# cmower/optas

Measured on AMD Instinct MI355X. Metric: MPC solves/sec (KUKA 7-DoF, T=50), higher is better.
Workload: dtype f64; 1 GPU; figure_eight_plan T=50 KUKA LWR end_effector_ball (BASELINE configs[1]) x 262144 perturbed instances per GPU (qc0 + U(-0.1,0.1)^7, seed=qc), solved to reduced-gradient tol 1e-08, max_iter 300; batch_per_gpu=262144, global_batch=262144, T=50, parallelism=dp1 (instances sharded, one RCCL broadcast of constants), rccl_world=1, hessian=hybrid, streams_per_gpu=2

## Files before the change

optas_amd/csrc/oh_api.hip:

```cpp
#include <algorithm>
#include <chrono>
#include <cmath>
#include <cstdlib>
#include <cstring>
#include <string>
#include <thread>
#include <utility>
#include <vector>

#include "oh_handle.h"

static thread_local std::string g_err;

int fail(int code, const std::string& msg) {
  g_err = msg;
  return code;
}

extern "C" int oh_specialize(oh_handle* h);
static bool spec_applies(const oh_handle* h);
static bool spec_tail_vel_applies(const oh_handle* h);
extern "C" const char* oh_last_error(void) { return g_err.c_str(); }
extern "C" const char* oh_version(void) { return "optas_hip 0.2 (gfx950)"; }
extern "C" int oh_abi_version(void) { return OH_ABI_VERSION; }

struct FieldOpt {
  const char* name;
  int Sched::*i;
  double Sched::*d = nullptr;
  bool flag = false;
  double get(const Sched& s) const { return d ? s.*d : s.*i; }
  void set(Sched& s, const double v) const { if (d) s.*d = v; else s.*i = flag ? v != 0.0 : (int)v; }
};
static const FieldOpt FIELD_OPTS[] = {
    {"tail_threshold", &Sched::tail_threshold}, {"free_pcr_max", &Sched::free_pcr_max}, {"compaction", &Sched::compaction, nullptr, true},
    {"compact_frac", nullptr, &Sched::compact_frac}, {"compact_sort", &Sched::compact_sort}, {"compact_carry", &Sched::compact_carry},
    {"compact_fused", &Sched::compact_fused, nullptr, true},
    {"tail_vel", &Sched::tail_vel}, {"lg_split", &Sched::lg_split}, {"tail_vel_threshold", &Sched::tail_vel_threshold},
    {"fuse_couple", &Sched::fuse_couple, nullptr, true}, {"sparse_check_below", &Sched::sparse_check_below}, {"specialize", &Sched::specialize},
    {"tq_check", &Sched::tq_check},
};
static const FieldOpt* field_opt(const std::string& name) {
  for (const FieldOpt& f : FIELD_OPTS)
    if (name == f.name) return &f;
  return nullptr;
}
static int set_option_impl(oh_handle* h, const std::string& name, double v) {
  Sched& sc = h->sch;
  if (name == "compact_frac") sc.compact_frac = sc.compact_frac_restart = v;
  else if (name == "specialize") sc.specialize = v == 0.0 ? OH_SPECIALIZE_NEVER : (v == 1.0 ? OH_SPECIALIZE_ALWAYS : OH_SPECIALIZE_AUTO);
  else if (name == "tq_check") sc.tq_check = v >= 1.0 ? (int)v : 1;
  else if (name == "batch_invariant") {
// ... 551 lines not shown
  for (int i = 1; i <= S; ++i) lo[i] = (int)((long long)a.B * i / S / 64 * 64);
  lo[S] = a.B;
  std::vector<LastSolve::Part> parts(S);
  const int rc = fan_out(h, S, [&](const int i, oh_handle* q, Tally& t) {
    parts[i] = {q, lo[i + 1] - lo[i]};
    return lane_solve(q, t, a.part((size_t)lo[i], parts[i].n, sh));
  });
  if (rc) return rc;
  rec->parts = parts;
  return OH_OK;
}

struct Traj {
  int B, N, NV, check_every, hard_cap;
  bool guarded, lead, prof, invariant;
  const FigSpec* spec;
  FreeSweep sweep;
  const double* p;
  double *x, *f, *kkt;
  int *iters, *status;
  int launched, compactions;
  size_t ne;
};
static FreeSweep free_sweep(oh_handle* h, const int nb, const bool start = false) {
  const int N = h->desc.ndof, nK = h->desc.T - h->P.t0;
  FreeSweep sw = FREE_SERIAL;
  if (!h->P.lock && batch_invariant(h) == 0.0 && nb <= h->sch.free_pcr_max && nK <= 128 && (N == 6 || N == 7)) {
    if (N == 7 && (int)optv(h, "free_bb") != 0) sw = FREE_BB;
    else sw = (nb <= (int)optv(h, "free_cp_max") && nK <= 64) ? FREE_CP : FREE_PCR;
  }
// ... 13 lines not shown
}
static bool check_after(const oh_handle* h, const Traj& r, const int it, const bool tail_ok) {
  return (it + 1) % ((!tail_ok && r.check_every == 1 && h->D.B <= h->sch.sparse_check_below) ? 8 : r.check_every) == 0;
}
static int look(oh_handle* h, const bool check, int* nrun) {
  *nrun = -1;
  if (!check) return OH_OK;
  hipStream_t s = h->stream;
  HIPCHK(hipMemcpyAsync(h->h_flag, h->D.n_running, sizeof(int), hipMemcpyDeviceToHost, s));
  HIPCHK(hipStreamSynchronize(s));
  *nrun = *h->h_flag;
  return OH_OK;
}
static void finalize(oh_handle* h, const Traj& r, const int only_done) {
  hipStream_t s = h->stream;
  if (r.spec && r.spec->finalize) {
    oh_launch_finalize(s, r.N, h->P, h->D, only_done, r.x, r.f, r.kkt, r.iters, r.status, 1);
    if (oh_spec_launch_finalize(*r.spec, s, h->P, h->D, only_done, r.f, r.kkt, r.iters, r.status) == hipSuccess) return;
    (void)hipGetLastError();
    oh_launch_finalize(s, r.N, h->P, h->D, only_done, r.x, r.f, r.kkt, r.iters, r.status, 2);
    return;
  }
  oh_launch_finalize(s, r.N, h->P, h->D, only_done, r.x, r.f, r.kkt, r.iters, r.status);
}
static int compact_batch(oh_handle* h, Traj& r, const int nrun, const int slot, const bool move) {
  hipStream_t s = h->stream;
  finalize(h, r, 1);
  if (r.guarded) oh_launch_guard_emit(s, h->P, h->D, h->GP, h->GB, r.NV, 1);
  oh_launch_scan_running(s, h->D, h->sch.compact_sort);
  if (move) {
// ... 15 lines not shown
    bool want = h->sch.specialize == OH_SPECIALIZE_ALWAYS || (h->sch.specialize == OH_SPECIALIZE_AUTO && r.B >= h->specialize_min_B);
    if (!want && h->sch.specialize == OH_SPECIALIZE_AUTO && !h->spec_cache_checked) {
      h->spec_cache_checked = true;
      want = oh_jit_figure8_cached(h->chain_host, h->desc.ndof);
    }
    if (want && oh_specialize(h) != OH_OK) h->spec_failed = true;
  }
  if (r.lead && (r.guarded || !h->desc.lock_orientation || h->desc.ndof != 6))
    return fail(OH_ERR_INVALID, "oh_solve_device: a parameterised lead joint is lowered for the orientation-locked family with 6 optimised joints, "
                                "without inequality rows");
  if (!r.guarded) h->D.fpsi = nullptr;
  else if (const int rc = ensure_guards(h)) return rc;
  r.sweep = free_sweep(h, r.B, true);
  r.NV = (r.guarded && h->GP.vel) ? 2 * r.N : 0;
  r.spec = spec_applies(h) ? h->spec : nullptr;
  r.check_every = optv(h, "check_every") >= 1.0 ? (int)optv(h, "check_every") : 1;
  r.hard_cap = 2 * h->desc.max_iter + 2 + 40 + 64;
  hipStream_t s = h->stream;
  if (r.prof) {
    const size_t need = 4 * (size_t)(2 * h->desc.max_iter + 44) + 64;
    while (h->prof_events.size() < need) {
      hipEvent_t e;
      HIPCHK(hipEventCreate(&e));
      h->prof_events.push_back(e);
    }
  }
  HIPCHK(hipEventRecord(h->ev0, s));
  HIPCHK(hipMemsetAsync(h->D.work, 0, 4 * sizeof(unsigned long long), s));
  if (!oh_launch_setup(s, r.N, h->P, h->D, x0, r.p)) return fail(OH_ERR_INVALID, "oh_solve_device: unsupported ndof");
  if (r.guarded) oh_launch_setup_guards(s, r.N, h->P, h->D, h->GP, h->GB, r.p);
  h->prof_tags.clear();
  return mark(h, r, 0);
}
static bool launch_tail(oh_handle* h, const Traj& r, const bool tail_vel, const int slot) {
  hipStream_t s = h->stream;
  if (tail_vel && h->spec && spec_tail_vel_applies(h)) return oh_spec_launch_tail_vel(*h->spec, s, h->P, h->D, h->GP, h->GB, slot) == hipSuccess;
  if (tail_vel) return oh_launch_tail_vel(s, r.N, h->P, h->D, h->GP, h->GB, slot);
  if (r.spec) return oh_spec_launch_tail(*r.spec, s, h->P, h->D, slot) == hipSuccess;
  return oh_launch_tail(s, r.N, h->P, h->D, slot);
}
static void launch_eval(oh_handle* h, const Traj& r, const int slot, const int part) {
  if (!r.spec) oh_launch_eval(h->stream, r.N, h->P, h->D, slot, part);
  else oh_spec_launch_eval(*r.spec, h->stream, h->P, h->D, slot, part);
}
// ... 122 lines not shown
    if (nrun == 0) break;
    if (nrun > 0 && h->sch.compaction && D.B >= 512 && (double)nrun <= h->sch.compact_frac_restart * (double)D.B) {
      if (const int rc = compact_batch(h, r, nrun, (it + 1) & 1, false)) return rc;
      sweep = free_sweep(h, D.B);
      h->free_sweeps_used |= 1 << (int)sweep;
      if (const int rc = mark(h, r, 0)) return rc;
    }
  }
  return OH_OK;
}
static int traj_epilogue(oh_handle* h, Traj& r) {
  hipStream_t s = h->stream;
  finalize(h, r, 0);
  if (r.guarded) oh_launch_guard_emit(s, h->P, h->D, h->GP, h->GB, r.NV, 0);
  h->D.B = r.B;
  if (r.guarded) oh_launch_guard_infeasible(s, r.N, h->P, h->D, h->GP, r.p, r.B, r.kkt, r.status);
  if (const int frc = finish_solve(h, r.launched)) return frc;
  unsigned long long work[3] = {0, 0, 0};
  HIPCHK(hipMemcpyAsync(work, h->D.work, sizeof(work), hipMemcpyDeviceToHost, s));
  HIPCHK(hipStreamSynchronize(s));
  h->timing[6] = (double)work[0];
  h->rejects = (double)work[1];
  h->tail_iters = (double)work[2];
  if (r.prof) {
    double ms[4] = {0, 0, 0, 0};
    int n[5] = {0, 0, 0, 0, 0};
    for (size_t i = 1; i < r.ne; ++i) {
      const int tag = h->prof_tags[i];
      float m = 0.f;
      if (tag) hipEventElapsedTime(&m, h->prof_events[i - 1], h->prof_events[i]);
// ... 345 lines not shown
```

optas_amd/csrc/oh_figure8_kernels.h:

```cpp
#pragma once
#include "oh_figure8_units.h"

template <int N, bool MOVE = false>
__device__ void retract_block(const FigParams& P, const FigBuffers& D, const int slot) {
  eval_unit<N, false, false, EVAL_RETRACT_ONLY, false, true, MOVE>(P, D, slot, blockIdx.x * blockDim.x + threadIdx.x, blockIdx.y + P.t0);
}
template <int N>
__device__ void finalize_block(const FigParams& P, const FigBuffers& D, const int only_done, double* __restrict__ f, double* __restrict__ kkt, int* __restrict__ iters,
                               int* __restrict__ status) {
  finalize_unit<N>(P, D, only_done, nullptr, f, kkt, iters, status, blockIdx.x * blockDim.x + threadIdx.x, blockIdx.y);
}
template <int N, bool ZC = false>
__device__ void evalb_block(const FigParams& P, const FigBuffers& D, const int slot) {
  if constexpr (ZC) {
    if (blockIdx.x == 0 && threadIdx.x == 0) *D.n_running = 0;
    const int Tn = P.T - P.t0;
    const int w = blockIdx.x;
    const int chunk = w / (8 * Tn), r = w - chunk * 8 * Tn;
    eval_unit<N, false, false, EVAL_ONLY, true>(P, D, slot, (chunk * 8 + (r & 7)) * blockDim.x + threadIdx.x, (r >> 3) + P.t0);
  } else {
    eval_unit<N, false, false, EVAL_ONLY, false>(P, D, slot, blockIdx.x * blockDim.x + threadIdx.x, blockIdx.y + P.t0);
  }
}

OH_DEV double bcast(const double v, const int lane) {
// ... 526 lines not shown
```

optas_amd/csrc/oh_figure8_units.h:

```cpp
#pragma once
#include "oh_figure8.h"

#define IDX(t, K, k) (((size_t)(t) * (K) + (k)) * Bp + b)
#define KNOT(arr, t, K) rowbuf((arr) + (size_t)(t) * (K) * (size_t)Bp)
#define RB(k) ((unsigned)(k) * rowB)
#define SPARE(k) (((size_t)t * N + (k)) * Bp + nb)



template <int N>
OH_DEV void setup_unit(const FigParams& P, const FigBuffers& D, const double* __restrict__ x0, const double* __restrict__ pin, const int b, const int tt) {
  const int Bp = D.Bp;
  if (b >= D.B) {
    if (b < Bp && tt == 0) D.status[b] = OH_STATUS_CONVERGED;
    return;
  }
  const oh_chain* ch = D.chain;
  double qc[N];
#pragma unroll
  for (int j = 0; j < N; ++j) qc[j] = pin[(size_t)b * P.np + j];
#pragma unroll
  for (int j = 0; j < N; ++j) {
    const double v = (tt < P.t0) ? qc[j] : x0[(size_t)b * P.nx + (size_t)tt * N + j];
    D.q[0][IDX(tt, N, j)] = v;
    D.q[1][IDX(tt, N, j)] = (tt < P.t0) ? qc[j] : 0.0;
  }
  if (ch->has_lead) D.lead[(size_t)tt * Bp + b] = pin[(size_t)b * P.np + N + 1 + tt];
  if (tt != 0) return;
  double R[9], p[3], z[N][3], pj[N][3];
  if (ch->has_lead) {
    double Rb[9], pb[3];
    lead_base(ch, pin[(size_t)b * P.np + N], Rb, pb);
    fk_chain<N, true>(ch, qc, R, p, z, pj, Rb, pb);
  } else {
    fk_chain<N>(ch, qc, R, p, z, pj);
  }
  double e[3], t[3], Re[9];
  mv3(R, ch->p_tool, t);
  e[0] = p[0] + t[0]; e[1] = p[1] + t[1]; e[2] = p[2] + t[2];
  mm3(R, ch->R_tool, Re);
#pragma unroll
  for (int i = 0; i < 3; ++i) D.ref[(size_t)i * Bp + b] = e[i];
#pragma unroll
// ... 1039 lines not shown
#pragma unroll
      for (int a = 0; a < NZ; ++a) {
        rb_st(KNOT(D.zstep, t, NZ), RB(a), lb, alpha * zz[a]);
        z2 += zz[a] * zz[a];
      }
    }
    D.pred[b] = -alpha * gd + 0.5 * alpha * alpha * (gd + mu * z2);
  }
  D.mu[b] = mu;
  D.iters[b] = iters + 1;
  return true;
}


template <int N>
OH_DEV void knot_multipliers(const FigParams& P, const FigBuffers& D, const int b, const int t, const int cur, double* out) {
  const int Bp = D.Bp;
  if (t < P.t0) {
    out[0] = out[1] = out[2] = out[3] = 0.0;
    return;
  }
  const oh_chain* ch = OH_CHAIN(D);
  const double* __restrict__ qs = D.q[cur];
  const double kap2 = 2.0 * P.kappa;
  double q[N], G[N];
  const bool last = (t == P.T - 1);
#pragma unroll
  for (int k = 0; k < N; ++k) {
    q[k] = qs[IDX(t, N, k)];
    if (P.zc) {
      G[k] = D.Gfull[cur][IDX(t, N, k)];
    } else {
      G[k] = D.g[cur][IDX(t, N, k)] + kap2 * (q[k] - qs[IDX(t - 1, N, k)]);
      if (!last) G[k] -= kap2 * (qs[IDX(t + 1, N, k)] - q[k]);
    }
  }
  double R[9], p[3], z[N][3], pj[N][3];
  if (ch->has_lead) {
    double Rb[9], pb[3];
    lead_base(ch, D.lead[(size_t)t * Bp + b], Rb, pb);
    fk_chain<N, true>(ch, q, R, p, z, pj, Rb, pb);
  } else {
    fk_chain<N>(ch, q, R, p, z, pj);
  }
  double S[6] = {1e-14, 0, 1e-14, 0, 0, 1e-14};
  double rhs[3] = {0, 0, 0};
#pragma unroll
  for (int k = 0; k < N; ++k) {
    if (ch->jtype[k] == 0) {
      S[0] += z[k][0] * z[k][0];
      S[1] += z[k][1] * z[k][0];
      S[2] += z[k][1] * z[k][1];
      S[3] += z[k][2] * z[k][0];
      S[4] += z[k][2] * z[k][1];
      S[5] += z[k][2] * z[k][2];
      rhs[0] -= z[k][0] * G[k]; rhs[1] -= z[k][1] * G[k]; rhs[2] -= z[k][2] * G[k];
    }
  }
  chol_packed<3>(S, 0.0);
  fsub<3>(S, rhs);
  bsub<3>(S, rhs);
  double quat[4] = {0, 0, 0, 1};
#pragma unroll
  for (int k = 0; k < N; ++k) {
    double qn[4];
    qmul(quat, ch->quat0[k], qn);
    if (ch->jtype[k] == 0) {
      double sh, chh;
      sincos_joint(0.5 * qs[IDX(0, N, k)], &sh, &chh);
      const double qa[4] = {sh * ch->axis[k][0], sh * ch->axis[k][1], sh * ch->axis[k][2], chh};
      qmul(qn, qa, quat);
    } else {
      quat[0] = qn[0]; quat[1] = qn[1]; quat[2] = qn[2]; quat[3] = qn[3];
    }
  }
  double qcq[4];
  qmul(quat, ch->quat_tool, qcq);
  const double o[4] = {rhs[0], rhs[1], rhs[2], 0.0};
  double nu[4];
  qmul(o, qcq, nu);
  out[0] = -2.0 * nu[0]; out[1] = -2.0 * nu[1]; out[2] = -2.0 * nu[2]; out[3] = -2.0 * nu[3];
}

template <int N>
OH_DEV void finalize_unit(const FigParams& P, const FigBuffers& D, int only_done, double* __restrict__ x, double* __restrict__ f,
                          double* __restrict__ kkt, int* __restrict__ iters, int* __restrict__ status, const int b, const int t) {
  const int Bp = D.Bp;
  if (b >= D.B) return;
  const int st = D.status[b];
  if (only_done && st < 0) return;
  const size_t ob = (size_t)D.orig[b];
  const int cur = D.cur[b];
  const double* __restrict__ qs = D.q[cur];
  if (x) {
    double* xb = x + ob * P.nx;
    double q0[N];
// ... 28 lines not shown
```

optas_amd/csrc/oh_handle.h:

```cpp
#pragma once
#include <hip/hip_runtime.h>

#include <array>
#include <map>
#include <string>
#include <vector>

#include "oh_kernels.h"
#include "oh_carve.h"
#include "oh_jit.h"

int fail(int code, const std::string& msg);

#define HIPCHK(expr)                                                                                   \
  do {                                                                                                 \
    hipError_t _e = (expr);                                                                            \
    if (_e != hipSuccess) {                                                                            \
      return fail(OH_ERR_HIP, std::string(#expr) + ": " + hipGetErrorString(_e));                     \
    }                                                                                                  \
  } while (0)

#define OH_PINNED_STAGE_BYTES (256 * 1024)

template <class T, bool PINNED = false>
// ... 28 lines not shown
struct Solve {
  int B;
  const double *x0, *p;
  double *x, *f, *kkt;
  int *iters, *status;
  Solve part(const size_t lo, const int n, const Shape& sh) const {
    const auto at = [lo](auto* q, const size_t per) -> decltype(q) { return q ? q + lo * per : nullptr; };
    return {n, at(x0, sh.nx), at(p, sh.npar), at(x, sh.nx), at(f, 1), at(kkt, 3), at(iters, 1), at(status, 1)};
  }
};

struct Sched {
  int compaction = 1;
  int compact_carry = 1;
  int compact_fused = 1;
  int tail_vel_threshold = 1 << 30;
  int lg_split = 1;
  int tail_vel = 1;
  int compact_sort = 1;
  double compact_frac = 0.97;
  double compact_frac_restart = 0.9;
  int tail_threshold = 16384;
  int sparse_check_below = 2048;
  int fuse_couple = 1;
  int free_pcr_max = 1536;
  int specialize = OH_SPECIALIZE_AUTO;
  int tq_check = 4;
  std::array<double, 4> inv_saved{1.0, 16384.0, 1.0, -2.0};
};

// ... 193 lines not shown
```

optas_amd/csrc/oh_jit.h:

```cpp
#pragma once
#include <string>
#include <vector>

#include "oh_kernels.h"

struct FigSpec {
  hipModule_t mod = nullptr;
  hipFunction_t retract = nullptr, retract_move = nullptr, evalb = nullptr, evalb_zc = nullptr, tail = nullptr, tail_vel = nullptr, finalize = nullptr;
  int n = 0;
  bool from_disk = false;
  double seconds = 0.0;
};
std::string oh_jit_figure8_source(const oh_chain& chain, int N);
int oh_jit_compile_cached(const std::string& src, std::vector<char>* code, bool* from_disk, std::string* err, bool ignore_disk = false);
int oh_jit_figure8(const oh_chain& chain, int N, const FigSpec** out, std::string* err);
bool oh_jit_figure8_cached(const oh_chain& chain, int N);
hipError_t oh_spec_launch_eval(const FigSpec& sp, hipStream_t s, const FigParams& P, const FigBuffers& D, int slot, int part);
hipError_t oh_spec_launch_tail(const FigSpec& sp, hipStream_t s, const FigParams& P, const FigBuffers& D, int slot);
hipError_t oh_spec_launch_finalize(const FigSpec& sp, hipStream_t s, FigParams P, FigBuffers D, int only_done, double* f, double* kkt, int* iters, int* status);
hipError_t oh_spec_launch_tail_vel(const FigSpec& sp, hipStream_t s, FigParams P, FigBuffers D, GuardParams GP, GuardBuffers GB, int slot);
bool oh_spec_kernel_info(const FigSpec& sp, const char* name, OhKernelInfo* out);

bool oh_jit_disk_lookup(const std::string& key_text, const char* prefix, std::vector<char>* code);
void oh_jit_disk_store(const std::string& key_text, const char* prefix, const std::vector<char>& code);
void oh_jit_disk_drop(const std::string& key_text, const char* prefix);

struct FkSpec {
  hipModule_t mod = nullptr;
  hipFunction_t soa = nullptr, aos = nullptr;
  int ndof = 0;
  bool from_disk = false;
  double seconds = 0.0;
};
std::string oh_jit_fkjac_source(const oh_chain& chain);
// ... 4 lines not shown
```

optas_amd/csrc/oh_jit.hip:

```cpp
#include <hip/hip_runtime.h>
#include <hip/hiprtc.h>
#include <sys/stat.h>
#include <unistd.h>

#include <chrono>
#include <cstdio>
#include <cstdlib>
#include <cstring>
#include <map>
#include <mutex>
#include <string>
#include <vector>

#include "oh_jit.h"
#include "oh_fkjac_unit.h"
#include "oh_jit_headers.h"

namespace {
std::mutex g_mutex;
std::map<unsigned long long, FigSpec*> g_specs;
std::map<unsigned long long, FkSpec*> g_fk_specs;

unsigned long long fnv1a(const std::string& s, unsigned long long h = 1469598103934665603ull) {
  for (unsigned char c : s) {
// ... 165 lines not shown
  s += "#define OH_RETRACT_PREFETCH " + std::to_string(OH_JIT_RETRACT_PREFETCH) + "\n";
#ifndef OH_JIT_ZC_EARLY
#define OH_JIT_ZC_EARLY 1
#endif
  s += "#define OH_ZC_EARLY " + std::to_string(OH_JIT_ZC_EARLY) + "\n";
  s += "#include \"oh_platform_gfx950.h\"\n";
  s += "#include \"oh_figure8_kernels.h\"\n";
  const std::string n = std::to_string(N);
  s += "extern \"C\" __global__ __launch_bounds__(256, 2) void oh_spec_retract(FigParams P, FigBuffers D, const int slot) { retract_block<" + n + ">(P, D, slot); }\n";
  s += "extern \"C\" __global__ __launch_bounds__(256, 2) void oh_spec_retract_move(FigParams P, FigBuffers D, const int slot) { retract_block<" + n + ", true>(P, D, slot); }\n";
  s += "extern \"C\" __global__ __launch_bounds__(256, 2) void oh_spec_evalb(FigParams P, FigBuffers D, const int slot) { evalb_block<" + n + ">(P, D, slot); }\n";
  s += "extern \"C\" __global__ __launch_bounds__(256, 2) void oh_spec_evalb_zc(FigParams P, FigBuffers D, const int slot) { evalb_block<" + n + ", true>(P, D, slot); }\n";
  s += "extern \"C\" __global__ __launch_bounds__(64) void oh_spec_tail(FigParams P, FigBuffers D, const int slot) { tail_block<" + n + ">(P, D, slot); }\n";
  s += "extern \"C\" __global__ __launch_bounds__(256) void oh_spec_finalize(FigParams P, FigBuffers D, const int only_done, double* f, double* kkt, int* iters, int* status) { finalize_block<" + n +
       ">(P, D, only_done, f, kkt, iters, status); }\n";
  s += "extern \"C\" __global__ __launch_bounds__(64) void oh_spec_tail_vel(FigParams P, FigBuffers D, GuardParams GP, GuardBuffers GB, const int slot) { tail_block<" + n +
       ", true>(P, D, slot, &GP, &GB); }\n";
  return s;
}

int oh_jit_compile_cached(const std::string& src, std::vector<char>* code, bool* from_disk, std::string* err, bool ignore_disk) {
  const std::string name = cache_name(src);
  const std::string dir = cache_dir();
  *from_disk = false;
  if (ignore_disk && !dir.empty()) remove((dir + "/" + name).c_str());
  if (!ignore_disk && !dir.empty() && read_file(dir + "/" + name, code)) {
    *from_disk = true;
    return 0;
  }
  if (compile(src, code, err)) return 1;
// ... 34 lines not shown
    return 0;
  }
  std::vector<char> code;
  bool from_disk = false;
  FigSpec* sp = new FigSpec();
  for (int attempt = 0;; ++attempt) {
    if (oh_jit_compile_cached(src, &code, &from_disk, err, attempt > 0)) {
      delete sp;
      return 1;
    }
    const char* what = nullptr;
    if (hipModuleLoadData(&sp->mod, code.data()) != hipSuccess) what = "hipModuleLoadData";
    else if (hipModuleGetFunction(&sp->retract, sp->mod, "oh_spec_retract") != hipSuccess || hipModuleGetFunction(&sp->evalb, sp->mod, "oh_spec_evalb") != hipSuccess ||
             hipModuleGetFunction(&sp->tail, sp->mod, "oh_spec_tail") != hipSuccess || hipModuleGetFunction(&sp->evalb_zc, sp->mod, "oh_spec_evalb_zc") != hipSuccess ||
             hipModuleGetFunction(&sp->tail_vel, sp->mod, "oh_spec_tail_vel") != hipSuccess || hipModuleGetFunction(&sp->finalize, sp->mod, "oh_spec_finalize") != hipSuccess ||
             hipModuleGetFunction(&sp->retract_move, sp->mod, "oh_spec_retract_move") != hipSuccess) {
      what = "hipModuleGetFunction";
      hipModuleUnload(sp->mod);
    }
    if (!what) break;
    (void)hipGetLastError();
    if (from_disk && attempt == 0) continue;
    *err = std::string(what) + " failed for the specialised figure-eight kernels";
    delete sp;
    return 1;
  }
  sp->n = N;
  sp->from_disk = from_disk;
  sp->seconds = std::chrono::duration<double>(std::chrono::steady_clock::now() - t0).count();
  g_specs.emplace(key, sp);
  *out = sp;
// ... 9 lines not shown
  hipError_t e = hipSuccess;
  if (part == 3) return launch3(sp.retract_move, ge, dim3(256), s, P, D, slot);
  if (part != 2) e = launch3(sp.retract, ge, dim3(256), s, P, D, slot);
  if (e == hipSuccess && part != 1) {
    if (P.zc) e = launch3(sp.evalb_zc, dim3((((D.B + 255) / 256) + 7) / 8 * 8 * (P.T - P.t0)), dim3(256), s, P, D, slot);
    else e = launch3(sp.evalb, ge, dim3(256), s, P, D, slot);
  }
  return e;
}
hipError_t oh_spec_launch_tail(const FigSpec& sp, hipStream_t s, const FigParams& P, const FigBuffers& D, int slot) {
  return launch3(sp.tail, dim3(D.B), dim3(64), s, P, D, slot);
}
hipError_t oh_spec_launch_finalize(const FigSpec& sp, hipStream_t s, FigParams P, FigBuffers D, int only_done, double* f, double* kkt, int* iters, int* status) {
  void* args[] = {&P, &D, &only_done, &f, &kkt, &iters, &status};
  return hipModuleLaunchKernel(sp.finalize, (D.B + 255) / 256, D.lam_h ? P.T : 1, 1, 256, 1, 1, 0, s, args, nullptr);
}
hipError_t oh_spec_launch_tail_vel(const FigSpec& sp, hipStream_t s, FigParams P, FigBuffers D, GuardParams GP, GuardBuffers GB, int slot) {
  void* args[] = {&P, &D, &GP, &GB, &slot};
  return hipModuleLaunchKernel(sp.tail_vel, D.B, 1, 1, 64, 1, 1, 0, s, args, nullptr);
}
bool oh_spec_kernel_info(const FigSpec& sp, const char* name, OhKernelInfo* out) {
  const std::string n(name);
  hipFunction_t f = n == "k_retract" ? sp.retract : n == "k_retract_move" ? sp.retract_move : n == "k_evalb" ? sp.evalb : n == "k_evalb_zc" ? sp.evalb_zc : n == "k_tail" ? sp.tail : n == "k_tail_vel" ? sp.tail_vel : nullptr;
  if (!f) return false;
  int v = 0, sc = 0, lds = 0;
  if (hipFuncGetAttribute(&v, HIP_FUNC_ATTRIBUTE_NUM_REGS, f) != hipSuccess) return false;
  hipFuncGetAttribute(&sc, HIP_FUNC_ATTRIBUTE_LOCAL_SIZE_BYTES, f);
  hipFuncGetAttribute(&lds, HIP_FUNC_ATTRIBUTE_SHARED_SIZE_BYTES, f);
  out->vgprs = v;
  out->scratch_bytes = sc;
// ... 77 lines not shown
```

optas_amd/csrc/oh_kernels.h:

```cpp
#pragma once
#include <hip/hip_runtime.h>

#include <string>
#include <vector>

#include "optas_hip.h"
#include "oh_types.h"

struct OhKernelInfo {
  int vgprs, scratch_bytes, lds_bytes, block, blocks_per_cu;
};
bool oh_kernel_info_figure8(const char* name, OhKernelInfo* out);
bool oh_kernel_info_fkjac(const char* name, OhKernelInfo* out);
bool oh_kernel_info_torque(const char* name, OhKernelInfo* out);
bool oh_kernel_info_linkkin(const char* name, OhKernelInfo* out);
bool oh_kernel_info_qp_block(const char* name, OhKernelInfo* out);

void oh_launch_fk_jac(hipStream_t s, bool soa, const oh_chain* d_chain, int n_chain, int ndof, int n, const double* q, double* pose, double* J);
struct OhLinkFrames {
  oh_chain link, base;
  int n_shared;
};
void oh_launch_link_kin(hipStream_t s, bool soa, const OhLinkFrames* d_frames, int n_link, int n, const double* q, const double* a3, const oh_link_out& out);
bool oh_launch_setup(hipStream_t s, int n, const FigParams& P, const FigBuffers& D, const double* x0, const double* p);
bool oh_launch_eval(hipStream_t s, int n, const FigParams& P, const FigBuffers& D, int slot, int part = 0);
bool oh_launch_carry(hipStream_t s, int n, const FigParams& P, const FigBuffers& D, int phase, int Bnew, int slot);
bool oh_launch_eval_lead(hipStream_t s, int n, const FigParams& P, const FigBuffers& D, int slot);
bool oh_launch_couple(hipStream_t s, int n, const FigParams& P, const FigBuffers& D, int slot);
bool oh_launch_couple_vel(hipStream_t s, int n, const FigParams& P, const FigBuffers& D, const GuardParams& GP, const GuardBuffers& GB, int slot);
bool oh_launch_step(hipStream_t s, int n, const FigParams& P, const FigBuffers& D, int slot);
bool oh_launch_eval_free(hipStream_t s, int n, const FigParams& P, const FigBuffers& D, int slot);
bool oh_launch_couple_free(hipStream_t s, int n, const FigParams& P, const FigBuffers& D, int slot);
bool oh_launch_couple_free_vel(hipStream_t s, int n, const FigParams& P, const FigBuffers& D, const GuardParams& GP, const GuardBuffers& GB, int slot);
enum FreeSweep { FREE_SERIAL, FREE_PCR, FREE_CP, FREE_BB, FREE_PERSIST };
bool oh_launch_step_free(hipStream_t s, int n, const FigParams& P, const FigBuffers& D, int slot, FreeSweep sweep);
void oh_launch_move_rows(hipStream_t s, void* arr, void* scr, int rows, int Bp, int B, int Bnew, const int* newidx, bool is_int);
void oh_launch_move_rows_live(hipStream_t s, double* a0, double* a1, double* scr, int rows, int Bp, int B, int Bnew, const int* newidx, const int* cur, const int* curn);
bool oh_launch_setup_guards(hipStream_t s, int n, const FigParams& P, const FigBuffers& D, const GuardParams& GP, const GuardBuffers& GB, const double* p);
void oh_launch_guard_infeasible(hipStream_t s, int n, const FigParams& P, const FigBuffers& D, const GuardParams& GP, const double* p, int B, double* kkt, int* status);
// ... 161 lines not shown
```

optas_amd/csrc/oh_kernels.hip:

```cpp
#include "oh_platform_gfx950.h"
#include "oh_figure8_kernels.h"
#include "oh_kernels.h"

#define OH_DISPATCH_N(n, call)         \
  switch (n) {                         \
    case 4: call(4); break;            \
    case 5: call(5); break;            \
    case 6: call(6); break;            \
    case 7: call(7); break;            \
    case 8: call(8); break;            \
    default: return false;             \
  }
#define OH_DISPATCH_N_ANY(n, call)     \
  switch (n) {                         \
    case 2: call(2); break;            \
    case 3: call(3); break;            \
    case 4: call(4); break;            \
    case 5: call(5); break;            \
    case 6: call(6); break;            \
    case 7: call(7); break;            \
    case 8: call(8); break;            \
    default: return false;             \
  }

template <int N>
__global__ __launch_bounds__(64) void k_setup(FigParams P, FigBuffers D, const double* __restrict__ x0, const double* __restrict__ pin) {
  setup_unit<N>(P, D, x0, pin, blockIdx.x * blockDim.x + threadIdx.x, blockIdx.y);
}
#ifndef OH_EVAL_WAVES
#define OH_EVAL_WAVES 1
#endif
template <int N>
__global__ __launch_bounds__(256, 2) void k_retract(FigParams P, FigBuffers D, const int slot) { retract_block<N>(P, D, slot); }
template <int N>
__global__ __launch_bounds__(256, 2) void k_evalb(FigParams P, FigBuffers D, const int slot) { evalb_block<N>(P, D, slot); }
template <int N>
__global__ __launch_bounds__(256, 2) void k_evalb_zc(FigParams P, FigBuffers D, const int slot) { evalb_block<N, true>(P, D, slot); }
template <int N>
__global__ __launch_bounds__(256, OH_EVAL_WAVES) void k_eval_lead(FigParams P, FigBuffers D, const int slot) {
  eval_unit<N, false, true>(P, D, slot, blockIdx.x * blockDim.x + threadIdx.x, blockIdx.y + P.t0);
}
bool oh_launch_eval_lead(hipStream_t s, int n, const FigParams& P, const FigBuffers& D, int slot) {
// ... 167 lines not shown
#pragma unroll
    for (int k = 0; k < SCAN_NB; ++k) v[k] = (tid >= off) ? cnt[k][tid - off] : 0;
    __syncthreads();
#pragma unroll
    for (int k = 0; k < SCAN_NB; ++k) cnt[k][tid] += v[k];
    __syncthreads();
  }
}
__global__ __launch_bounds__(SCAN_TPB) void k_scan_count(FigBuffers D, const int sort, const int chunk, int* __restrict__ blk) {
  __shared__ int cnt[SCAN_NB][SCAN_TPB];
  int c[SCAN_NB], lo, hi;
  scan_block(D, sort, chunk, c, cnt, lo, hi);
  if (threadIdx.x < SCAN_NB) blk[threadIdx.x * SCAN_MAXBLK + blockIdx.x] = cnt[threadIdx.x][SCAN_TPB - 1];
}
__global__ __launch_bounds__(SCAN_MAXBLK) void k_scan_offsets(FigBuffers D, const int nblk, int* __restrict__ blk) {
  __shared__ int sc[SCAN_MAXBLK];
  __shared__ int carry;
  const int tid = threadIdx.x;
  if (tid == 0) carry = 0;
  __syncthreads();
  for (int k = 0; k < SCAN_NB; ++k) {
    const int mine = (tid < nblk) ? blk[k * SCAN_MAXBLK + tid] : 0;
    sc[tid] = mine;
    __syncthreads();
    for (int off = 1; off < SCAN_MAXBLK; off <<= 1) {
      const int v = (tid >= off) ? sc[tid - off] : 0;
      __syncthreads();
      sc[tid] += v;
      __syncthreads();
    }
    if (tid < nblk) blk[k * SCAN_MAXBLK + tid] = carry + sc[tid] - mine;
    __syncthreads();
    if (tid == 0) carry += sc[SCAN_MAXBLK - 1];
    __syncthreads();
  }
  if (tid == 0) *D.n_new = carry;
}
__global__ __launch_bounds__(SCAN_TPB) void k_scan_assign(FigBuffers D, const int sort, const int chunk, const int* __restrict__ blk) {
  __shared__ int cnt[SCAN_NB][SCAN_TPB];
  int c[SCAN_NB], lo, hi;
  scan_block(D, sort, chunk, c, cnt, lo, hi);
  int pos[SCAN_NB];
#pragma unroll
  for (int k = 0; k < SCAN_NB; ++k) pos[k] = blk[k * SCAN_MAXBLK + blockIdx.x] + cnt[k][threadIdx.x] - c[k];
  for (int b = lo; b < hi; ++b) {
    if (D.status[b] < 0) {
      const int kb = scan_class(D, b, sort);
      int p = 0;
#pragma unroll
// ... 124 lines not shown
    D.nun[b] = ts[(size_t)16 * Bp + b];
    D.f_cur[b] = ts[(size_t)17 * Bp + b];
    D.pred[b] = ts[(size_t)18 * Bp + b];
    D.stat[b] = ts[(size_t)19 * Bp + b];
    D.feas[b] = ts[(size_t)20 * Bp + b];
    D.cur[b] = 1 - slot;
    D.first[b] = restart ? 1 : 0;
    D.skip[b] = 0;
    D.polish[b] = (!restart && (flags & 2)) ? ((flags & 4) ? 2 : 1) : 0;
    D.stale[b] = restart ? 0 : 1;
    D.status[b] = -1;
  }
}

template <int N>
static void launch_setup_t(hipStream_t s, const FigParams& P, const FigBuffers& D, const double* x0, const double* p) {
  hipLaunchKernelGGL(k_setup<N>, dim3((D.B + 63) / 64, P.T), dim3(64), 0, s, P, D, x0, p);
}
template <int N>
static void launch_eval_t(hipStream_t s, const FigParams& P, const FigBuffers& D, int slot, int part) {
  const dim3 ge((D.B + 255) / 256, P.T - P.t0);
  if (part != 2) hipLaunchKernelGGL(k_retract<N>, ge, dim3(256), 0, s, P, D, slot);
  if (part != 1) {
    if (P.zc) hipLaunchKernelGGL(k_evalb_zc<N>, dim3((((D.B + 255) / 256) + 7) / 8 * 8 * (P.T - P.t0)), dim3(256), 0, s, P, D, slot);
    else hipLaunchKernelGGL(k_evalb<N>, ge, dim3(256), 0, s, P, D, slot);
  }
}
template <int N>
static void launch_carry_t(hipStream_t s, const FigParams& P, const FigBuffers& D, int phase, int Bnew, int slot) {
  if (phase == 0) hipLaunchKernelGGL(k_carry_gather<N>, dim3((D.B + 255) / 256, P.T), dim3(256), 0, s, P, D, slot);
  else if (phase == 2) hipLaunchKernelGGL((k_carry_gather<N, true>), dim3((D.B + 255) / 256, P.t0 > 1 ? P.t0 : 1), dim3(256), 0, s, P, D, slot);
  else hipLaunchKernelGGL(k_carry_scatter<N>, dim3((Bnew + 255) / 256), dim3(256), 0, s, P, D, Bnew, slot);
}
// ... 41 lines not shown
  }
}
template <int N>
static void launch_finalize_t(hipStream_t s, const FigParams& P, const FigBuffers& D, int only_done, double* x, double* f, double* kkt,
                              int* iters, int* status, const int parts) {
  if (x && (parts & 1)) hipLaunchKernelGGL(k_finalize_x<N>, dim3((D.B + 63) / 64, (P.T + 7) / 8), dim3(256), 0, s, P, D, only_done, x);
  if (!(parts & 2)) return;
  hipLaunchKernelGGL(k_finalize<N>, dim3((D.B + 255) / 256, D.lam_h ? P.T : 1), dim3(256), 0, s, P, D, only_done, (double*)nullptr, f, kkt, iters, status);
}
template <int N>
static void launch_compact_t(hipStream_t s, const FigParams& P, const FigBuffers& D, int phase, int Bnew, int slot) {
  if (phase == 0) hipLaunchKernelGGL(k_compact_gather<N>, dim3((D.B + 255) / 256, P.T), dim3(256), 0, s, P, D);
  else hipLaunchKernelGGL(k_compact_scatter<N>, dim3((Bnew + 255) / 256, P.T), dim3(256), 0, s, P, D, Bnew, slot);
}

bool oh_launch_setup(hipStream_t s, int n, const FigParams& P, const FigBuffers& D, const double* x0, const double* p) {
#define C(NN) launch_setup_t<NN>(s, P, D, x0, p)
  OH_DISPATCH_N_ANY(n, C)
#undef C
  return true;
}
bool oh_launch_eval(hipStream_t s, int n, const FigParams& P, const FigBuffers& D, int slot, int part) {
#define C(NN) launch_eval_t<NN>(s, P, D, slot, part)
  OH_DISPATCH_N(n, C)
#undef C
  return true;
}
bool oh_launch_carry(hipStream_t s, int n, const FigParams& P, const FigBuffers& D, int phase, int Bnew, int slot) {
#define C(NN) launch_carry_t<NN>(s, P, D, phase, Bnew, slot)
  OH_DISPATCH_N(n, C)
#undef C
  return true;
}
// ... 131 lines not shown
```

Baseline: 3.259 million solves/s.

## Recompute multipliers densely from final x; tile setup loads; parallelize offset scan

Result: no change. 3.268 million solves/s, median of 2 (+0.3%).

```diff
diff --git a/optas_amd/csrc/oh_api.hip b/optas_amd/csrc/oh_api.hip
--- a/optas_amd/csrc/oh_api.hip
+++ b/optas_amd/csrc/oh_api.hip
@@ -36,6 +36,7 @@
     {"tail_threshold", &Sched::tail_threshold}, {"free_pcr_max", &Sched::free_pcr_max}, {"compaction", &Sched::compaction, nullptr, true},
     {"compact_frac", nullptr, &Sched::compact_frac}, {"compact_sort", &Sched::compact_sort}, {"compact_carry", &Sched::compact_carry},
     {"compact_fused", &Sched::compact_fused, nullptr, true},
+    {"dense_multipliers", &Sched::dense_multipliers, nullptr, true}, {"setup_tiled", &Sched::setup_tiled, nullptr, true},
     {"tail_vel", &Sched::tail_vel}, {"lg_split", &Sched::lg_split}, {"tail_vel_threshold", &Sched::tail_vel_threshold},
     {"fuse_couple", &Sched::fuse_couple, nullptr, true}, {"sparse_check_below", &Sched::sparse_check_below}, {"specialize", &Sched::specialize},
     {"tq_check", &Sched::tq_check},
@@ -617,6 +618,7 @@
 struct Traj {
   int B, N, NV, check_every, hard_cap;
   bool guarded, lead, prof, invariant;
+  bool dense;
   const FigSpec* spec;
   FreeSweep sweep;
   const double* p;
@@ -660,6 +662,13 @@
 }
 static void finalize(oh_handle* h, const Traj& r, const int only_done) {
   hipStream_t s = h->stream;
+  if (r.dense) {
+    FigBuffers Dn = h->D;
+    Dn.lam_h = nullptr;
+    oh_launch_finalize(s, r.N, h->P, h->D, only_done, r.x, r.f, r.kkt, r.iters, r.status, 1);
+    oh_launch_finalize(s, r.N, h->P, Dn, only_done, r.x, r.f, r.kkt, r.iters, r.status, 2);
+    return;
+  }
   if (r.spec && r.spec->finalize) {
     oh_launch_finalize(s, r.N, h->P, h->D, only_done, r.x, r.f, r.kkt, r.iters, r.status, 1);
     if (oh_spec_launch_finalize(*r.spec, s, h->P, h->D, only_done, r.f, r.kkt, r.iters, r.status) == hipSuccess) return;
@@ -705,6 +714,7 @@
   r.sweep = free_sweep(h, r.B, true);
   r.NV = (r.guarded && h->GP.vel) ? 2 * r.N : 0;
   r.spec = spec_applies(h) ? h->spec : nullptr;
+  r.dense = h->sch.dense_multipliers && h->P.lock && !r.guarded && !r.lead && r.x && h->D.lam_h;
   r.check_every = optv(h, "check_every") >= 1.0 ? (int)optv(h, "check_every") : 1;
   r.hard_cap = 2 * h->desc.max_iter + 2 + 40 + 64;
   hipStream_t s = h->stream;
@@ -718,7 +728,7 @@
   }
   HIPCHK(hipEventRecord(h->ev0, s));
   HIPCHK(hipMemsetAsync(h->D.work, 0, 4 * sizeof(unsigned long long), s));
-  if (!oh_launch_setup(s, r.N, h->P, h->D, x0, r.p)) return fail(OH_ERR_INVALID, "oh_solve_device: unsupported ndof");
+  if (!oh_launch_setup(s, r.N, h->P, h->D, x0, r.p, h->sch.setup_tiled && !r.lead)) return fail(OH_ERR_INVALID, "oh_solve_device: unsupported ndof");
   if (r.guarded) oh_launch_setup_guards(s, r.N, h->P, h->D, h->GP, h->GB, r.p);
   h->prof_tags.clear();
   return mark(h, r, 0);
@@ -871,6 +881,12 @@
   finalize(h, r, 0);
   if (r.guarded) oh_launch_guard_emit(s, h->P, h->D, h->GP, h->GB, r.NV, 0);
   h->D.B = r.B;
+  if (r.dense) {
+    if (!(r.spec && r.spec->multipliers_x && oh_spec_launch_multipliers_x(*r.spec, s, h->P, h->D, r.B, r.x) == hipSuccess)) {
+      (void)hipGetLastError();
+      oh_launch_multipliers_x(s, r.N, h->P, h->D, r.B, r.x);
+    }
+  }
   if (r.guarded) oh_launch_guard_infeasible(s, r.N, h->P, h->D, h->GP, r.p, r.B, r.kkt, r.status);
   if (const int frc = finish_solve(h, r.launched)) return frc;
   unsigned long long work[3] = {0, 0, 0};
diff --git a/optas_amd/csrc/oh_figure8_kernels.h b/optas_amd/csrc/oh_figure8_kernels.h
--- a/optas_amd/csrc/oh_figure8_kernels.h
+++ b/optas_amd/csrc/oh_figure8_kernels.h
@@ -9,6 +9,77 @@
 __device__ void finalize_block(const FigParams& P, const FigBuffers& D, const int only_done, double* __restrict__ f, double* __restrict__ kkt, int* __restrict__ iters,
                                int* __restrict__ status) {
   finalize_unit<N>(P, D, only_done, nullptr, f, kkt, iters, status, blockIdx.x * blockDim.x + threadIdx.x, blockIdx.y);
+}
+template <int N>
+__device__ void multipliers_block(const FigParams& P, const FigBuffers& D, const int B, const double* __restrict__ x) {
+  constexpr int TK = 8, ROWS = (TK + 2) * N, KPW = TK / 4;
+  __shared__ double tile[ROWS][65];
+  __shared__ double refs[16][64];
+  const oh_chain* ch = OH_CHAIN(D);
+  const int lane = threadIdx.x & 63, w = threadIdx.x >> 6;
+  const int b0 = blockIdx.x * 64, b = b0 + lane, T = P.T;
+  if (w == 0 && b < B) {
+    double q0[N], Rc[9], pc[3], qcq[4];
+#pragma unroll
+    for (int j = 0; j < N; ++j) q0[j] = x[(size_t)b * P.nx + j];
+    instance_refs<N>(ch, q0, Rc, pc, qcq);
+#pragma unroll
+    for (int i = 0; i < 9; ++i) refs[i][lane] = Rc[i];
+#pragma unroll
+    for (int i = 0; i < 3; ++i) refs[9 + i][lane] = pc[i];
+#pragma unroll
+    for (int i = 0; i < 4; ++i) refs[12 + i][lane] = qcq[i];
+  }
+  __syncthreads();
+  double Rc[9], pc[3], qcq[4];
+#pragma unroll
+  for (int i = 0; i < 9; ++i) Rc[i] = refs[i][lane];
+#pragma unroll
+  for (int i = 0; i < 3; ++i) pc[i] = refs[9 + i][lane];
+#pragma unroll
+  for (int i = 0; i < 4; ++i) qcq[i] = refs[12 + i][lane];
+  for (int ts = 0; ts < T; ts += TK) {
+    const int lo = ts > 0 ? ts - 1 : 0, hi = min(ts + TK, T - 1);
+    const int nrows = (hi - lo + 1) * N, nk = min(TK, T - ts);
+    for (int i = w; i < 64; i += 4) {
+      if (b0 + i >= B) break;
+      const double* xb = x + (size_t)(b0 + i) * P.nx + (size_t)lo * N;
+      for (int idx = lane; idx < nrows; idx += 64) tile[idx][i] = xb[idx];
+    }
+    __syncthreads();
+    double o[KPW][4];
+#pragma unroll
+    for (int kk = 0; kk < KPW; ++kk) {
+      const int t = ts + w + 4 * kk;
+      o[kk][0] = o[kk][1] = o[kk][2] = o[kk][3] = 0.0;
+      if (t < T && t >= P.t0 && b < B) {
+        double qm[N], q[N], qp[N];
+        const int r = (t - lo) * N;
+#pragma unroll
+        for (int j = 0; j < N; ++j) {
+          qm[j] = tile[r - N + j][lane];
+          q[j] = tile[r + j][lane];
+          qp[j] = (t < T - 1) ? tile[r + N + j][lane] : 0.0;
+        }
+        knot_multipliers_x<N>(ch, P, t, qm, q, qp, Rc, pc, qcq, o[kk]);
+      }
+    }
+    __syncthreads();
+#pragma unroll
+    for (int kk = 0; kk < KPW; ++kk) {
+      const int t = ts + w + 4 * kk;
+      if (t < T) {
+#pragma unroll
+        for (int c = 0; c < 4; ++c) tile[(t - ts) * 4 + c][lane] = o[kk][c];
+      }
+    }
+    __syncthreads();
+    for (int i = w; i < 64; i += 4) {
+      if (b0 + i >= B) break;
+      if (lane < nk * 4) D.lam_h[((size_t)(b0 + i) * T + ts) * 4 + lane] = tile[lane][i];
+    }
+    __syncthreads();
+  }
 }
 template <int N, bool ZC = false>
 __device__ void evalb_block(const FigParams& P, const FigBuffers& D, const int slot) {
diff --git a/optas_amd/csrc/oh_figure8_units.h b/optas_amd/csrc/oh_figure8_units.h
--- a/optas_amd/csrc/oh_figure8_units.h
+++ b/optas_amd/csrc/oh_figure8_units.h
@@ -8,6 +8,8 @@
 
 
 
+template <int N>
+OH_DEV void setup_instance(const FigParams& P, const FigBuffers& D, const double* __restrict__ pin, const int b, const double (&qc)[N]);
 template <int N>
 OH_DEV void setup_unit(const FigParams& P, const FigBuffers& D, const double* __restrict__ x0, const double* __restrict__ pin, const int b, const int tt) {
   const int Bp = D.Bp;
@@ -26,7 +28,12 @@
     D.q[1][IDX(tt, N, j)] = (tt < P.t0) ? qc[j] : 0.0;
   }
   if (ch->has_lead) D.lead[(size_t)tt * Bp + b] = pin[(size_t)b * P.np + N + 1 + tt];
-  if (tt != 0) return;
+  if (tt == 0) setup_instance<N>(P, D, pin, b, qc);
+}
+template <int N>
+OH_DEV void setup_instance(const FigParams& P, const FigBuffers& D, const double* __restrict__ pin, const int b, const double (&qc)[N]) {
+  const int Bp = D.Bp;
+  const oh_chain* ch = D.chain;
   double R[9], p[3], z[N][3], pj[N][3];
   if (ch->has_lead) {
     double Rb[9], pb[3];
@@ -1096,35 +1103,25 @@
 
 
 template <int N>
-OH_DEV void knot_multipliers(const FigParams& P, const FigBuffers& D, const int b, const int t, const int cur, double* out) {
-  const int Bp = D.Bp;
-  if (t < P.t0) {
-    out[0] = out[1] = out[2] = out[3] = 0.0;
-    return;
-  }
-  const oh_chain* ch = OH_CHAIN(D);
-  const double* __restrict__ qs = D.q[cur];
-  const double kap2 = 2.0 * P.kappa;
-  double q[N], G[N];
-  const bool last = (t == P.T - 1);
+OH_DEV void quat_of_chain(const oh_chain* __restrict__ ch, const double (&q0)[N], double (&qcq)[4]) {
+  double quat[4] = {0, 0, 0, 1};
 #pragma unroll
   for (int k = 0; k < N; ++k) {
-    q[k] = qs[IDX(t, N, k)];
-    if (P.zc) {
-      G[k] = D.Gfull[cur][IDX(t, N, k)];
+    double qn[4];
+    qmul(quat, ch->quat0[k], qn);
+    if (ch->jtype[k] == 0) {
+      double sh, chh;
+      sincos_joint(0.5 * q0[k], &sh, &chh);
+      const double qa[4] = {sh * ch->axis[k][0], sh * ch->axis[k][1], sh * ch->axis[k][2], chh};
+      qmul(qn, qa, quat);
     } else {
-      G[k] = D.g[cur][IDX(t, N, k)] + kap2 * (q[k] - qs[IDX(t - 1, N, k)]);
-      if (!last) G[k] -= kap2 * (qs[IDX(t + 1, N, k)] - q[k]);
-    }
-  }
-  double R[9], p[3], z[N][3], pj[N][3];
-  if (ch->has_lead) {
-    double Rb[9], pb[3];
-    lead_base(ch, D.lead[(size_t)t * Bp + b], Rb, pb);
-    fk_chain<N, true>(ch, q, R, p, z, pj, Rb, pb);
-  } else {
-    fk_chain<N>(ch, q, R, p, z, pj);
-  }
+      quat[0] = qn[0]; quat[1] = qn[1]; quat[2] = qn[2]; quat[3] = qn[3];
+    }
+  }
+  qmul(quat, ch->quat_tool, qcq);
+}
+template <int N>
+OH_DEV void multipliers_from_G(const oh_chain* __restrict__ ch, const double (&z)[N][3], const double (&G)[N], const double (&qcq)[4], double* out) {
   double S[6] = {1e-14, 0, 1e-14, 0, 0, 1e-14};
   double rhs[3] = {0, 0, 0};
 #pragma unroll
@@ -1142,26 +1139,94 @@
   chol_packed<3>(S, 0.0);
   fsub<3>(S, rhs);
   bsub<3>(S, rhs);
-  double quat[4] = {0, 0, 0, 1};
-#pragma unroll
-  for (int k = 0; k < N; ++k) {
-    double qn[4];
-    qmul(quat, ch->quat0[k], qn);
-    if (ch->jtype[k] == 0) {
-      double sh, chh;
-      sincos_joint(0.5 * qs[IDX(0, N, k)], &sh, &chh);
-      const double qa[4] = {sh * ch->axis[k][0], sh * ch->axis[k][1], sh * ch->axis[k][2], chh};
-      qmul(qn, qa, quat);
-    } else {
-      quat[0] = qn[0]; quat[1] = qn[1]; quat[2] = qn[2]; quat[3] = qn[3];
-    }
-  }
-  double qcq[4];
-  qmul(quat, ch->quat_tool, qcq);
   const double o[4] = {rhs[0], rhs[1], rhs[2], 0.0};
   double nu[4];
   qmul(o, qcq, nu);
   out[0] = -2.0 * nu[0]; out[1] = -2.0 * nu[1]; out[2] = -2.0 * nu[2]; out[3] = -2.0 * nu[3];
+}
+
+template <int N>
+OH_DEV void knot_multipliers(const FigParams& P, const FigBuffers& D, const int b, const int t, const int cur, double* out) {
+  const int Bp = D.Bp;
+  if (t < P.t0) {
+    out[0] = out[1] = out[2] = out[3] = 0.0;
+    return;
+  }
+  const oh_chain* ch = OH_CHAIN(D);
+  const double* __restrict__ qs = D.q[cur];
+  const double kap2 = 2.0 * P.kappa;
+  double q[N], G[N];
+  const bool last = (t == P.T - 1);
+#pragma unroll
+  for (int k = 0; k < N; ++k) {
+    q[k] = qs[IDX(t, N, k)];
+    if (P.zc) {
+      G[k] = D.Gfull[cur][IDX(t, N, k)];
+    } else {
+      G[k] = D.g[cur][IDX(t, N, k)] + kap2 * (q[k] - qs[IDX(t - 1, N, k)]);
+      if (!last) G[k] -= kap2 * (qs[IDX(t + 1, N, k)] - q[k]);
+    }
+  }
+  double R[9], p[3], z[N][3], pj[N][3];
+  if (ch->has_lead) {
+    double Rb[9], pb[3];
+    lead_base(ch, D.lead[(size_t)t * Bp + b], Rb, pb);
+    fk_chain<N, true>(ch, q, R, p, z, pj, Rb, pb);
+  } else {
+    fk_chain<N>(ch, q, R, p, z, pj);
+  }
+  double q0[N], qcq[4];
+#pragma unroll
+  for (int k = 0; k < N; ++k) q0[k] = qs[IDX(0, N, k)];
+  quat_of_chain<N>(ch, q0, qcq);
+  multipliers_from_G<N>(ch, z, G, qcq, out);
+}
+
+template <int N>
+OH_DEV void instance_refs(const oh_chain* __restrict__ ch, const double (&q0)[N], double (&Rc)[9], double (&pc)[3], double (&qcq)[4]) {
+  double R[9], p[3], z[N][3], pj[N][3], t[3];
+  fk_chain<N>(ch, q0, R, p, z, pj);
+  mv3(R, ch->p_tool, t);
+  pc[0] = p[0] + t[0]; pc[1] = p[1] + t[1]; pc[2] = p[2] + t[2];
+  mm3(R, ch->R_tool, Rc);
+  quat_of_chain<N>(ch, q0, qcq);
+}
+template <int N>
+OH_DEV void knot_multipliers_x(const oh_chain* __restrict__ ch, const FigParams& P, const int t, const double (&qm)[N], const double (&q)[N], const double (&qp)[N],
+                               const double (&Rc)[9], const double (&pc)[3], const double (&qcq)[4], double* out) {
+  if (t < P.t0) {
+    out[0] = out[1] = out[2] = out[3] = 0.0;
+    return;
+  }
+  double R[9], p[3], z[N][3], pj[N][3];
+  fk_chain<N>(ch, q, R, p, z, pj);
+  double e[3], tv[3];
+  mv3(R, ch->p_tool, tv);
+  e[0] = p[0] + tv[0]; e[1] = p[1] + tv[1]; e[2] = p[2] + tv[2];
+  const double l[3] = {P.local_path[3 * t], P.local_path[3 * t + 1], P.local_path[3 * t + 2]};
+  double r[3];
+  if (P.path_in_frame) mv3(Rc, l, r);
+  else { r[0] = l[0]; r[1] = l[1]; r[2] = l[2]; }
+  r[0] += pc[0] - e[0]; r[1] += pc[1] - e[1]; r[2] += pc[2] - e[2];
+  const double w = P.w_path, kap2 = 2.0 * P.kappa;
+  const bool last = (t == P.T - 1);
+  double G[N];
+#pragma unroll
+  for (int k = 0; k < N; ++k) {
+    double Jp[3];
+    if (ch->jtype[k] == 0) {
+      const double d[3] = {e[0] - pj[k][0], e[1] - pj[k][1], e[2] - pj[k][2]};
+      cross3(z[k], d, Jp);
+    } else {
+      Jp[0] = z[k][0]; Jp[1] = z[k][1]; Jp[2] = z[k][2];
+    }
+    const double g = -2.0 * w * dot3(Jp, r);
+    const double dm = q[k] - qm[k];
+    double c = kap2 * dm;
+    if (!last) c -= kap2 * (qp[k] - q[k]);
+    G[k] = g + c;
+  }
+  multipliers_from_G<N>(ch, z, G, qcq, out);
 }
 
 template <int N>
diff --git a/optas_amd/csrc/oh_handle.h b/optas_amd/csrc/oh_handle.h
--- a/optas_amd/csrc/oh_handle.h
+++ b/optas_amd/csrc/oh_handle.h
@@ -66,6 +66,8 @@
   int compaction = 1;
   int compact_carry = 1;
   int compact_fused = 1;
+  int dense_multipliers = 1;
+  int setup_tiled = 1;
   int tail_vel_threshold = 1 << 30;
   int lg_split = 1;
   int tail_vel = 1;
diff --git a/optas_amd/csrc/oh_jit.h b/optas_amd/csrc/oh_jit.h
--- a/optas_amd/csrc/oh_jit.h
+++ b/optas_amd/csrc/oh_jit.h
@@ -6,7 +6,7 @@
 
 struct FigSpec {
   hipModule_t mod = nullptr;
-  hipFunction_t retract = nullptr, retract_move = nullptr, evalb = nullptr, evalb_zc = nullptr, tail = nullptr, tail_vel = nullptr, finalize = nullptr;
+  hipFunction_t retract = nullptr, retract_move = nullptr, evalb = nullptr, evalb_zc = nullptr, tail = nullptr, tail_vel = nullptr, finalize = nullptr, multipliers_x = nullptr;
   int n = 0;
   bool from_disk = false;
   double seconds = 0.0;
@@ -18,6 +18,7 @@
 hipError_t oh_spec_launch_eval(const FigSpec& sp, hipStream_t s, const FigParams& P, const FigBuffers& D, int slot, int part);
 hipError_t oh_spec_launch_tail(const FigSpec& sp, hipStream_t s, const FigParams& P, const FigBuffers& D, int slot);
 hipError_t oh_spec_launch_finalize(const FigSpec& sp, hipStream_t s, FigParams P, FigBuffers D, int only_done, double* f, double* kkt, int* iters, int* status);
+hipError_t oh_spec_launch_multipliers_x(const FigSpec& sp, hipStream_t s, FigParams P, FigBuffers D, int B, const double* x);
 hipError_t oh_spec_launch_tail_vel(const FigSpec& sp, hipStream_t s, FigParams P, FigBuffers D, GuardParams GP, GuardBuffers GB, int slot);
 bool oh_spec_kernel_info(const FigSpec& sp, const char* name, OhKernelInfo* out);
 
diff --git a/optas_amd/csrc/oh_jit.hip b/optas_amd/csrc/oh_jit.hip
--- a/optas_amd/csrc/oh_jit.hip
+++ b/optas_amd/csrc/oh_jit.hip
@@ -203,6 +203,7 @@
   s += "extern \"C\" __global__ __launch_bounds__(64) void oh_spec_tail(FigParams P, FigBuffers D, const int slot) { tail_block<" + n + ">(P, D, slot); }\n";
   s += "extern \"C\" __global__ __launch_bounds__(256) void oh_spec_finalize(FigParams P, FigBuffers D, const int only_done, double* f, double* kkt, int* iters, int* status) { finalize_block<" + n +
        ">(P, D, only_done, f, kkt, iters, status); }\n";
+  s += "extern \"C\" __global__ __launch_bounds__(256) void oh_spec_multipliers_x(FigParams P, FigBuffers D, const int B, const double* x) { multipliers_block<" + n + ">(P, D, B, x); }\n";
   s += "extern \"C\" __global__ __launch_bounds__(64) void oh_spec_tail_vel(FigParams P, FigBuffers D, GuardParams GP, GuardBuffers GB, const int slot) { tail_block<" + n +
        ", true>(P, D, slot, &GP, &GB); }\n";
   return s;
@@ -267,7 +268,8 @@
     else if (hipModuleGetFunction(&sp->retract, sp->mod, "oh_spec_retract") != hipSuccess || hipModuleGetFunction(&sp->evalb, sp->mod, "oh_spec_evalb") != hipSuccess ||
              hipModuleGetFunction(&sp->tail, sp->mod, "oh_spec_tail") != hipSuccess || hipModuleGetFunction(&sp->evalb_zc, sp->mod, "oh_spec_evalb_zc") != hipSuccess ||
              hipModuleGetFunction(&sp->tail_vel, sp->mod, "oh_spec_tail_vel") != hipSuccess || hipModuleGetFunction(&sp->finalize, sp->mod, "oh_spec_finalize") != hipSuccess ||
-             hipModuleGetFunction(&sp->retract_move, sp->mod, "oh_spec_retract_move") != hipSuccess) {
+             hipModuleGetFunction(&sp->retract_move, sp->mod, "oh_spec_retract_move") != hipSuccess ||
+             hipModuleGetFunction(&sp->multipliers_x, sp->mod, "oh_spec_multipliers_x") != hipSuccess) {
       what = "hipModuleGetFunction";
       hipModuleUnload(sp->mod);
     }
@@ -307,6 +309,10 @@
 hipError_t oh_spec_launch_finalize(const FigSpec& sp, hipStream_t s, FigParams P, FigBuffers D, int only_done, double* f, double* kkt, int* iters, int* status) {
   void* args[] = {&P, &D, &only_done, &f, &kkt, &iters, &status};
   return hipModuleLaunchKernel(sp.finalize, (D.B + 255) / 256, D.lam_h ? P.T : 1, 1, 256, 1, 1, 0, s, args, nullptr);
+}
+hipError_t oh_spec_launch_multipliers_x(const FigSpec& sp, hipStream_t s, FigParams P, FigBuffers D, int B, const double* x) {
+  void* args[] = {&P, &D, &B, &x};
+  return hipModuleLaunchKernel(sp.multipliers_x, (B + 63) / 64, 1, 1, 256, 1, 1, 0, s, args, nullptr);
 }
 hipError_t oh_spec_launch_tail_vel(const FigSpec& sp, hipStream_t s, FigParams P, FigBuffers D, GuardParams GP, GuardBuffers GB, int slot) {
   void* args[] = {&P, &D, &GP, &GB, &slot};
diff --git a/optas_amd/csrc/oh_kernels.h b/optas_amd/csrc/oh_kernels.h
--- a/optas_amd/csrc/oh_kernels.h
+++ b/optas_amd/csrc/oh_kernels.h
@@ -22,7 +22,8 @@
   int n_shared;
 };
 void oh_launch_link_kin(hipStream_t s, bool soa, const OhLinkFrames* d_frames, int n_link, int n, const double* q, const double* a3, const oh_link_out& out);
-bool oh_launch_setup(hipStream_t s, int n, const FigParams& P, const FigBuffers& D, const double* x0, const double* p);
+bool oh_launch_setup(hipStream_t s, int n, const FigParams& P, const FigBuffers& D, const double* x0, const double* p, bool tiled = false);
+bool oh_launch_multipliers_x(hipStream_t s, int n, const FigParams& P, const FigBuffers& D, int B, const double* x);
 bool oh_launch_eval(hipStream_t s, int n, const FigParams& P, const FigBuffers& D, int slot, int part = 0);
 bool oh_launch_carry(hipStream_t s, int n, const FigParams& P, const FigBuffers& D, int phase, int Bnew, int slot);
 bool oh_launch_eval_lead(hipStream_t s, int n, const FigParams& P, const FigBuffers& D, int slot);
diff --git a/optas_amd/csrc/oh_kernels.hip b/optas_amd/csrc/oh_kernels.hip
--- a/optas_amd/csrc/oh_kernels.hip
+++ b/optas_amd/csrc/oh_kernels.hip
@@ -26,6 +26,38 @@
 template <int N>
 __global__ __launch_bounds__(64) void k_setup(FigParams P, FigBuffers D, const double* __restrict__ x0, const double* __restrict__ pin) {
   setup_unit<N>(P, D, x0, pin, blockIdx.x * blockDim.x + threadIdx.x, blockIdx.y);
+}
+template <int N>
+__global__ __launch_bounds__(256) void k_setup_x(FigParams P, FigBuffers D, const double* __restrict__ x0, const double* __restrict__ pin) {
+  constexpr int TK = 8, ROWS = TK * N;
+  __shared__ double tile[ROWS][65];
+  const int Bp = D.Bp;
+  const int lane = threadIdx.x & 63, w = threadIdx.x >> 6;
+  const int b0 = blockIdx.x * 64, b = b0 + lane, ts = blockIdx.y * TK;
+  const int nrows = min(TK, P.T - ts) * N;
+  for (int i = w; i < 64; i += 4) {
+    if (b0 + i >= D.B) break;
+    const double* xb = x0 + (size_t)(b0 + i) * P.nx + (size_t)ts * N;
+    if (lane < nrows) tile[lane][i] = xb[lane];
+  }
+  __syncthreads();
+  if (b >= D.B) {
+    if (b < Bp && ts == 0 && w == 0) D.status[b] = OH_STATUS_CONVERGED;
+    return;
+  }
+  for (int row = w; row < nrows; row += 4) {
+    const int t = ts + row / N, j = row % N;
+    const bool pinned = t < P.t0;
+    const double qcj = pinned ? pin[(size_t)b * P.np + j] : 0.0;
+    D.q[0][IDX(t, N, j)] = pinned ? qcj : tile[row][lane];
+    D.q[1][IDX(t, N, j)] = qcj;
+  }
+  if (ts == 0 && w == 0) {
+    double qc[N];
+#pragma unroll
+    for (int j = 0; j < N; ++j) qc[j] = pin[(size_t)b * P.np + j];
+    setup_instance<N>(P, D, pin, b, qc);
+  }
 }
 #ifndef OH_EVAL_WAVES
 #define OH_EVAL_WAVES 1
@@ -223,25 +255,26 @@
   if (threadIdx.x < SCAN_NB) blk[threadIdx.x * SCAN_MAXBLK + blockIdx.x] = cnt[threadIdx.x][SCAN_TPB - 1];
 }
 __global__ __launch_bounds__(SCAN_MAXBLK) void k_scan_offsets(FigBuffers D, const int nblk, int* __restrict__ blk) {
-  __shared__ int sc[SCAN_MAXBLK];
-  __shared__ int carry;
+  __shared__ int sc[SCAN_NB][SCAN_MAXBLK];
   const int tid = threadIdx.x;
-  if (tid == 0) carry = 0;
+  int mine[SCAN_NB];
+#pragma unroll
+  for (int k = 0; k < SCAN_NB; ++k) sc[k][tid] = mine[k] = (tid < nblk) ? blk[k * SCAN_MAXBLK + tid] : 0;
   __syncthreads();
+  for (int off = 1; off < SCAN_MAXBLK; off <<= 1) {
+    int v[SCAN_NB];
+#pragma unroll
+    for (int k = 0; k < SCAN_NB; ++k) v[k] = (tid >= off) ? sc[k][tid - off] : 0;
+    __syncthreads();
+#pragma unroll
+    for (int k = 0; k < SCAN_NB; ++k) sc[k][tid] += v[k];
+    __syncthreads();
+  }
+  int carry = 0;
+#pragma unroll
   for (int k = 0; k < SCAN_NB; ++k) {
-    const int mine = (tid < nblk) ? blk[k * SCAN_MAXBLK + tid] : 0;
-    sc[tid] = mine;
-    __syncthreads();
-    for (int off = 1; off < SCAN_MAXBLK; off <<= 1) {
-      const int v = (tid >= off) ? sc[tid - off] : 0;
-      __syncthreads();
-      sc[tid] += v;
-      __syncthreads();
-    }
-    if (tid < nblk) blk[k * SCAN_MAXBLK + tid] = carry + sc[tid] - mine;
-    __syncthreads();
-    if (tid == 0) carry += sc[SCAN_MAXBLK - 1];
-    __syncthreads();
+    if (tid < nblk) blk[k * SCAN_MAXBLK + tid] = carry + sc[k][tid] - mine[k];
+    carry += sc[k][SCAN_MAXBLK - 1];
   }
   if (tid == 0) *D.n_new = carry;
 }
@@ -396,9 +429,12 @@
 }
 
 template <int N>
-static void launch_setup_t(hipStream_t s, const FigParams& P, const FigBuffers& D, const double* x0, const double* p) {
-  hipLaunchKernelGGL(k_setup<N>, dim3((D.B + 63) / 64, P.T), dim3(64), 0, s, P, D, x0, p);
-}
+static void launch_setup_t(hipStream_t s, const FigParams& P, const FigBuffers& D, const double* x0, const double* p, const bool tiled) {
+  if (tiled) hipLaunchKernelGGL(k_setup_x<N>, dim3((D.B + 63) / 64, (P.T + 7) / 8), dim3(256), 0, s, P, D, x0, p);
+  else hipLaunchKernelGGL(k_setup<N>, dim3((D.B + 63) / 64, P.T), dim3(64), 0, s, P, D, x0, p);
+}
+template <int N>
+__global__ __launch_bounds__(256) void k_multipliers_x(FigParams P, FigBuffers D, const int B, const double* __restrict__ x) { multipliers_block<N>(P, D, B, x); }
 template <int N>
 static void launch_eval_t(hipStream_t s, const FigParams& P, const FigBuffers& D, int slot, int part) {
   const dim3 ge((D.B + 255) / 256, P.T - P.t0);
@@ -470,9 +506,15 @@
   else hipLaunchKernelGGL(k_compact_scatter<N>, dim3((Bnew + 255) / 256, P.T), dim3(256), 0, s, P, D, Bnew, slot);
 }
 
-bool oh_launch_setup(hipStream_t s, int n, const FigParams& P, const FigBuffers& D, const double* x0, const double* p) {
-#define C(NN) launch_setup_t<NN>(s, P, D, x0, p)
+bool oh_launch_setup(hipStream_t s, int n, const FigParams& P, const FigBuffers& D, const double* x0, const double* p, bool tiled) {
+#define C(NN) launch_setup_t<NN>(s, P, D, x0, p, tiled)
   OH_DISPATCH_N_ANY(n, C)
+#undef C
+  return true;
+}
+bool oh_launch_multipliers_x(hipStream_t s, int n, const FigParams& P, const FigBuffers& D, int B, const double* x) {
+#define C(NN) hipLaunchKernelGGL(k_multipliers_x<NN>, dim3((B + 63) / 64), dim3(256), 0, s, P, D, B, x)
+  OH_DISPATCH_N(n, C)
 #undef C
   return true;
 }
```
